# 4paradigm/OpenEmbedding

Hardware: NVIDIA H100
Metric: samples/sec (whole job, device-timed, max over ranks) deepfm Criteo dim 64 (higher is better)
Workload: dtype bf16

## Files before the change

openembedding_b200/csrc/cuda/gemm_wgmma.cu:

```cuda
#include <cuda.h>
#include <cuda_bf16.h>
#include <cuda_runtime.h>
#include "pdl.cuh"
#include <stdint.h>
#include <stdio.h>
#include <stdlib.h>
#include <string.h>

#include <string>
#include <vector>
#include <algorithm>

namespace {

constexpr int BM = 128, BK = 64;
constexpr int A_BYTES = BM * BK * 2;
template <int BN> constexpr int stages_for() { return BN == 64 ? 4 : 3; }
constexpr int NUM_CONSUMER_WARPS = 8;
constexpr int PRODUCER_WARP = NUM_CONSUMER_WARPS;
constexpr int NUM_THREADS = 32 * (NUM_CONSUMER_WARPS + 1);

enum EpiMode : int { EPI_FWD = 0, EPI_DX = 1, EPI_DW = 2, EPI_DX_FM = 3 };

struct GemmEpi {
    int mode, relu, ones_col, fm_cols;
    int M, N, D, mn_major;
    void* out; long long ldo;
    __nv_bfloat16* outT; long long ldoT;
    const __nv_bfloat16* mask; long long ldmask;
    const float* dlogit; const float* S; const float* emb; long long ldemb;
    int swap, mc;
    unsigned long long* dbg;
};

__device__ __forceinline__ uint32_t smem_u32(const void* p) { return (uint32_t)__cvta_generic_to_shared(p); }

__device__ __forceinline__ void mbar_init(uint64_t* b, uint32_t n) {
    asm volatile("mbarrier.init.shared::cta.b64 [%0], %1;" ::"r"(smem_u32(b)), "r"(n) : "memory");
}
__device__ __forceinline__ void mbar_expect_tx(uint64_t* b, uint32_t bytes) {
    asm volatile("mbarrier.arrive.expect_tx.shared::cta.b64 _, [%0], %1;" ::"r"(smem_u32(b)), "r"(bytes) : "memory");
}
__device__ __forceinline__ void mbar_arrive(uint64_t* b) {
    asm volatile("mbarrier.arrive.shared::cta.b64 _, [%0];" ::"r"(smem_u32(b)) : "memory");
}
__device__ __forceinline__ void mbar_arrive_cluster(uint64_t* b, uint32_t cta) {
    asm volatile("{\n\t.reg .b32 ra;\n\tmapa.shared::cluster.u32 ra, %0, %1;\n\t"
                 "mbarrier.arrive.release.cluster.shared::cluster.b64 _, [ra];\n\t}"
                 ::"r"(smem_u32(b)), "r"(cta) : "memory");
}
__device__ __forceinline__ bool mbar_try(uint64_t* b, uint32_t parity) {
    uint32_t ok;
    asm volatile("{\n\t.reg .pred p;\n\tmbarrier.try_wait.parity.shared::cta.b64 p, [%1], %2;\n\tselp.u32 %0, 1, 0, p;\n\t}"
                 : "=r"(ok) : "r"(smem_u32(b)), "r"(parity) : "memory");
    return ok != 0;
}
__device__ unsigned int g_pipeline_timeouts;
__device__ __forceinline__ bool mbar_wait(uint64_t* b, uint32_t parity) {
    for (uint32_t it = 0; it < (1u << 24); ++it)
        if (mbar_try(b, parity)) return true;
    atomicAdd(&g_pipeline_timeouts, 1u);
    return false;
}
__device__ __forceinline__ void tma_load_2d(void* smem_dst, const CUtensorMap* map, uint64_t* bar, int c0, int c1) {
    asm volatile("cp.async.bulk.tensor.2d.shared::cluster.global.mbarrier::complete_tx::bytes [%0], [%1, {%3, %4}], [%2];"
                 ::"r"(smem_u32(smem_dst)), "l"(map), "r"(smem_u32(bar)), "r"(c0), "r"(c1) : "memory");
}
__device__ __forceinline__ void tma_load_2d_mc(void* smem_dst, const CUtensorMap* map, uint64_t* bar, int c0, int c1, uint16_t mask) {
    asm volatile("cp.async.bulk.tensor.2d.shared::cluster.global.mbarrier::complete_tx::bytes.multicast::cluster [%0], [%1, {%4, %5}], [%2], %3;"
                 ::"r"(smem_u32(smem_dst)), "l"(map), "r"(smem_u32(bar)), "h"(mask), "r"(c0), "r"(c1) : "memory");
}
__device__ __forceinline__ void cluster_sync_all() {
    asm volatile("barrier.cluster.arrive.release.aligned;" ::: "memory");
    asm volatile("barrier.cluster.wait.acquire.aligned;" ::: "memory");
}
__device__ __forceinline__ void named_bar_sync(int id, int threads) {
    asm volatile("bar.sync %0, %1;" ::"r"(id), "r"(threads) : "memory");
}

__device__ __forceinline__ uint64_t gmma_desc(uint32_t smem_addr, uint32_t lbo_bytes) {
    uint64_t d = 0;
    d |= (uint64_t)((smem_addr & 0x3FFFFu) >> 4);
    d |= (uint64_t)((lbo_bytes >> 4) & 0x3FFFu) << 16;
    d |= (uint64_t)(1024 >> 4) << 32;
    d |= (uint64_t)1 << 62;
    return d;
}
__device__ __forceinline__ void wgmma_fence() { asm volatile("wgmma.fence.sync.aligned;" ::: "memory"); }
__device__ __forceinline__ void wgmma_commit() { asm volatile("wgmma.commit_group.sync.aligned;" ::: "memory"); }
template <int N>
__device__ __forceinline__ void wgmma_wait() { asm volatile("wgmma.wait_group.sync.aligned %0;" ::"n"(N) : "memory"); }
template <int R>
__device__ __forceinline__ void acc_fence(float (&d)[R]) {
#pragma unroll
    for (int i = 0; i < R; ++i) asm volatile("" : "+f"(d[i])::"memory");
}

template <int TRANS>
__device__ __forceinline__ void wgmma_n64(float (&d)[32], uint64_t da, uint64_t db, uint32_t scale_d) {
    asm volatile("{\n\t.reg .pred p;\n\tsetp.ne.b32 p, %34, 0;\n\t"
                 "wgmma.mma_async.sync.aligned.m64n64k16.f32.bf16.bf16 {"
                 "%0, %1, %2, %3, %4, %5, %6, %7, %8, %9, %10, %11, %12, %13, %14, %15, "
                 "%16, %17, %18, %19, %20, %21, %22, %23, %24, %25, %26, %27, %28, %29, %30, %31"
                 "}, %32, %33, p, 1, 1, %35, %35;\n\t}"
                 : "+f"(d[0]), "+f"(d[1]), "+f"(d[2]), "+f"(d[3]), "+f"(d[4]), "+f"(d[5]), "+f"(d[6]), "+f"(d[7]),
                   "+f"(d[8]), "+f"(d[9]), "+f"(d[10]), "+f"(d[11]), "+f"(d[12]), "+f"(d[13]), "+f"(d[14]), "+f"(d[15]),
                   "+f"(d[16]), "+f"(d[17]), "+f"(d[18]), "+f"(d[19]), "+f"(d[20]), "+f"(d[21]), "+f"(d[22]), "+f"(d[23]),
                   "+f"(d[24]), "+f"(d[25]), "+f"(d[26]), "+f"(d[27]), "+f"(d[28]), "+f"(d[29]), "+f"(d[30]), "+f"(d[31])
                 : "l"(da), "l"(db), "r"(scale_d), "n"(TRANS));
}
template <int TRANS>
__device__ __forceinline__ void wgmma_n128(float (&d)[64], uint64_t da, uint64_t db, uint32_t scale_d) {
    asm volatile("{\n\t.reg .pred p;\n\tsetp.ne.b32 p, %66, 0;\n\t"
                 "wgmma.mma_async.sync.aligned.m64n128k16.f32.bf16.bf16 {"
                 "%0, %1, %2, %3, %4, %5, %6, %7, %8, %9, %10, %11, %12, %13, %14, %15, "
                 "%16, %17, %18, %19, %20, %21, %22, %23, %24, %25, %26, %27, %28, %29, %30, %31, "
                 "%32, %33, %34, %35, %36, %37, %38, %39, %40, %41, %42, %43, %44, %45, %46, %47, "
                 "%48, %49, %50, %51, %52, %53, %54, %55, %56, %57, %58, %59, %60, %61, %62, %63"
                 "}, %64, %65, p, 1, 1, %67, %67;\n\t}"
                 : "+f"(d[0]), "+f"(d[1]), "+f"(d[2]), "+f"(d[3]), "+f"(d[4]), "+f"(d[5]), "+f"(d[6]), "+f"(d[7]),
                   "+f"(d[8]), "+f"(d[9]), "+f"(d[10]), "+f"(d[11]), "+f"(d[12]), "+f"(d[13]), "+f"(d[14]), "+f"(d[15]),
                   "+f"(d[16]), "+f"(d[17]), "+f"(d[18]), "+f"(d[19]), "+f"(d[20]), "+f"(d[21]), "+f"(d[22]), "+f"(d[23]),
                   "+f"(d[24]), "+f"(d[25]), "+f"(d[26]), "+f"(d[27]), "+f"(d[28]), "+f"(d[29]), "+f"(d[30]), "+f"(d[31]),
                   "+f"(d[32]), "+f"(d[33]), "+f"(d[34]), "+f"(d[35]), "+f"(d[36]), "+f"(d[37]), "+f"(d[38]), "+f"(d[39]),
                   "+f"(d[40]), "+f"(d[41]), "+f"(d[42]), "+f"(d[43]), "+f"(d[44]), "+f"(d[45]), "+f"(d[46]), "+f"(d[47]),
                   "+f"(d[48]), "+f"(d[49]), "+f"(d[50]), "+f"(d[51]), "+f"(d[52]), "+f"(d[53]), "+f"(d[54]), "+f"(d[55]),
                   "+f"(d[56]), "+f"(d[57]), "+f"(d[58]), "+f"(d[59]), "+f"(d[60]), "+f"(d[61]), "+f"(d[62]), "+f"(d[63])
                 : "l"(da), "l"(db), "r"(scale_d), "n"(TRANS));
}
template <int BN, int TRANS>
__device__ __forceinline__ void wgmma_stage(float (&acc)[BN / 2], uint32_t a0, uint32_t b0, int g, bool first) {
#pragma unroll
    for (int k = 0; k < BK / 16; ++k) {
        const uint64_t da = TRANS ? gmma_desc(a0 + g * 8192 + k * 2048, 8192) : gmma_desc(a0 + g * 8192 + k * 32, 16);
        const uint64_t db = TRANS ? gmma_desc(b0 + k * 2048, 8192) : gmma_desc(b0 + k * 32, 16);
        const uint32_t sd = (first && k == 0) ? 0u : 1u;
        if constexpr (BN == 64) wgmma_n64<TRANS>(acc, da, db, sd);
        else wgmma_n128<TRANS>(acc, da, db, sd);
    }
}

template <int BN>
__device__ __forceinline__ void mma_tile(float (&acc)[BN / 2], const uint8_t* sA, const uint8_t* sB, uint64_t* full,
                                         uint64_t* empty, int stages, uint32_t kiter, int nkb, bool mn_major, int g,
                                         int C) {
    constexpr int B_BYTES = BN * BK * 2;
    const int lane = threadIdx.x & 31;
#pragma unroll
    for (int j = 0; j < BN / 2; ++j) acc[j] = 0.f;
    auto release = [&](uint32_t it) {
        const int s = it % stages;
        if (C > 1) { if (lane < C) mbar_arrive_cluster(&empty[s], (uint32_t)lane); }
        else if (lane == 0) mbar_arrive(&empty[s]);
    };
    for (int i = 0; i < nkb; ++i) {
        const uint32_t it = kiter + i;
        const int s = it % stages;
        mbar_wait(&full[s], (it / stages) & 1u);
        const uint32_t a0 = smem_u32(sA + s * A_BYTES), b0 = smem_u32(sB + s * B_BYTES);
        wgmma_fence();
        if (mn_major) wgmma_stage<BN, 1>(acc, a0, b0, g, i == 0);
        else wgmma_stage<BN, 0>(acc, a0, b0, g, i == 0);
        wgmma_commit();
        if (i > 0) {
            wgmma_wait<1>();
            acc_fence(acc);
            release(it - 1);
        }
    }
    wgmma_wait<0>();
    acc_fence(acc);
    if (nkb > 0) release(kiter + nkb - 1);
}

template <int BN>
__device__ __forceinline__ void epilogue_tile(const GemmEpi& E, float (&acc)[BN / 2], int m_blk, int n_blk, int g,
                                              uint8_t* stage, int qstride, const CUtensorMap* tO, const CUtensorMap* tT) {
    const int mode = E.mode, relu = E.relu, ones_col = E.ones_col, fm_cols = E.fm_cols, N = E.N, D = E.D;
    const bool has_t = E.outT != nullptr;
    const int t = threadIdx.x & 127, w = t >> 5, l = t & 31;
    const bool f32out = (mode == EPI_DW || mode == EPI_DX_FM);
    const int q = 2 * g + (w >> 1);
    uint8_t* wstage = stage + q * qstride;
    uint8_t* tstage = wstage + BN * 128;
    constexpr int LOOK = BN == 64 ? 4 : 1;
#pragma unroll
    for (int i = 0; i < 2; ++i) {
        const int qrow = (w & 1) * 16 + (l >> 2) + 8 * i;
        const int row = m_blk * BM + q * 32 + qrow;
        const bool rv = row < E.M;
        const bool fm_row = mode == EPI_DX_FM && rv && n_blk * BN < fm_cols;
        const float dl = fm_row ? __ldg(E.dlogit + row) : 0.f;
        const __nv_bfloat16* mrow = E.mask + (size_t)row * E.ldmask;
        const float* erow = E.emb + (size_t)row * E.ldemb;
        const float* sb = E.S + (size_t)row * D;
#pragma unroll
        for (int j0 = 0; j0 < BN / 8; j0 += LOOK) {
            float4 v[LOOK];
#pragma unroll
            for (int jj = 0; jj < LOOK; ++jj) {
                const int n = n_blk * BN + 8 * (j0 + jj) + 2 * (l & 3);
                v[jj] = make_float4(0.f, 0.f, 0.f, 0.f);
                if (mode == EPI_DX) {
                    if (rv && n < N) {
                        const float2 mk = __bfloat1622float2(__ldg(reinterpret_cast<const __nv_bfloat162*>(mrow + n)));
                        v[jj].x = mk.x; v[jj].y = mk.y;
                    }
                } else if (fm_row && n < fm_cols) {
                    const float2 e2 = __ldg(reinterpret_cast<const float2*>(erow + n));
                    v[jj] = make_float4(e2.x, e2.y, __ldg(sb + n % D), __ldg(sb + (n + 1) % D));
                }
            }
#pragma unroll
            for (int jj = 0; jj < LOOK; ++jj) {
                const int j = j0 + jj;
                const int c = 8 * j + 2 * (l & 3);
                const int n = n_blk * BN + c;
                float x[2] = {acc[4 * j + 2 * i], acc[4 * j + 2 * i + 1]};
                if (mode == EPI_FWD) {
#pragma unroll
                    for (int u = 0; u < 2; ++u) {
                        if (relu) x[u] = fmaxf(x[u], 0.f);
                        if (n + u == ones_col) x[u] = 1.f;
                        if (n + u >= N) x[u] = 0.f;
                    }
                } else if (mode == EPI_DX) {
                    const float mv[2] = {v[jj].x, v[jj].y};
#pragma unroll
                    for (int u = 0; u < 2; ++u)
                        if (!rv || !(mv[u] > 0.f) || n + u == ones_col || n + u >= N) x[u] = 0.f;
                } else if (fm_row && n < fm_cols) {
                    x[0] += dl * (v[jj].z - v[jj].x);
                    x[1] += dl * (v[jj].w - v[jj].y);
                }
                if (f32out) {
                    const int cc = c & 31;
                    *reinterpret_cast<float2*>(wstage + (c >> 5) * 4096 + qrow * 128 + ((((cc >> 2) ^ (qrow & 7))) << 4) + (cc & 3) * 4) =
                        make_float2(x[0], x[1]);
                } else {
                    const int cc = c & 63;
                    *reinterpret_cast<__nv_bfloat162*>(wstage + (c >> 6) * 4096 + qrow * 128 + ((((cc >> 3) ^ (qrow & 7))) << 4) + (cc & 7) * 2) =
                        __floats2bfloat162_rn(x[0], x[1]);
                    if (has_t) {
                        *reinterpret_cast<__nv_bfloat16*>(tstage + c * 64 + qrow * 2) = __float2bfloat16_rn(x[0]);
                        *reinterpret_cast<__nv_bfloat16*>(tstage + (c + 1) * 64 + qrow * 2) = __float2bfloat16_rn(x[1]);
                    }
                }
            }
        }
    }
    asm volatile("fence.proxy.async.shared::cta;" ::: "memory");
    named_bar_sync(2 + g, 128);
    if (t == 0) {
        if (E.fm_cols != -7) {
#pragma unroll 1
            for (int qq = 2 * g; qq < 2 * g + 2; ++qq) {
                const int row0 = m_blk * BM + qq * 32;
                uint8_t* ws = stage + qq * qstride;
                if (f32out) {
#pragma unroll 1
                    for (int h = 0; h < BN / 32; ++h) {
                        const int n0 = n_blk * BN + 32 * h;
                        if (E.mode == EPI_DW)
                            asm volatile("cp.reduce.async.bulk.tensor.2d.global.shared::cta.add.tile.bulk_group [%0, {%2, %3}], [%1];"
                                         ::"l"(tO), "r"(smem_u32(ws + h * 4096)), "r"(n0), "r"(row0) : "memory");
                        else
                            asm volatile("cp.async.bulk.tensor.2d.global.shared::cta.bulk_group [%0, {%2, %3}], [%1];"
                                         ::"l"(tO), "r"(smem_u32(ws + h * 4096)), "r"(n0), "r"(row0) : "memory");
                    }
                } else {
#pragma unroll 1
                    for (int h = 0; h < BN / 64; ++h)
                        asm volatile("cp.async.bulk.tensor.2d.global.shared::cta.bulk_group [%0, {%2, %3}], [%1];"
                                     ::"l"(tO), "r"(smem_u32(ws + h * 4096)), "r"(n_blk * BN + 64 * h), "r"(row0) : "memory");
                    if (E.outT)
                        asm volatile("cp.async.bulk.tensor.2d.global.shared::cta.bulk_group [%0, {%2, %3}], [%1];"
                                     ::"l"(tT), "r"(smem_u32(ws + BN * 128)), "r"(row0), "r"(n_blk * BN) : "memory");
                }
            }
        }
        asm volatile("cp.async.bulk.commit_group;" ::: "memory");
    }
}

template <int BN>
__global__ void __launch_bounds__(NUM_THREADS, 2)
exb_gemm_wgmma_kernel(const __grid_constant__ CUtensorMap tmA, const __grid_constant__ CUtensorMap tmB,
                      const __grid_constant__ CUtensorMap tmO, const __grid_constant__ CUtensorMap tmT,
                      GemmEpi E, int num_k_blocks, int k_blocks_per_split) {
    static_assert(BN == 64 || BN == 128, "tile width");
    constexpr int STAGES = stages_for<BN>();
    constexpr int B_BYTES = BN * BK * 2;
    constexpr int QSTAGE = BN * 128 + BN * 64;
    static_assert(4 * QSTAGE <= STAGES * (A_BYTES + B_BYTES), "epilogue staging aliases the stage memory");
    extern __shared__ __align__(1024) uint8_t smem_raw[];
    uint8_t* smem = smem_raw + ((1024u - (smem_u32(smem_raw) & 1023u)) & 1023u);
    uint8_t* sA = smem;
    uint8_t* sB = smem + STAGES * A_BYTES;
    uint64_t* full = reinterpret_cast<uint64_t*>(sB + STAGES * B_BYTES);
    uint64_t* empty = full + STAGES;

    exb::pdl_trigger();
    const int warp = threadIdx.x >> 5, lane = threadIdx.x & 31;
    const int m_blk = E.swap ? blockIdx.y : blockIdx.x, n_blk = E.swap ? blockIdx.x : blockIdx.y;
    const bool dbg = E.dbg != nullptr && blockIdx.x == 0 && blockIdx.y == 0 && blockIdx.z == 0;
#define GSTAMP(i) do { if (dbg) { unsigned long long _t; asm volatile("mov.u64 %0, %%globaltimer;" : "=l"(_t)); E.dbg[i] = _t; } } while (0)
    if (threadIdx.x == 0) GSTAMP(0);
    const int kb0 = blockIdx.z * k_blocks_per_split;
    const int kb1 = min(num_k_blocks, kb0 + k_blocks_per_split);
    const int nkb = kb1 - kb0;
    const int C = E.mc > 1 ? E.mc : 1;
    uint32_t crank = 0;
    if (C > 1) asm volatile("mov.u32 %0, %%cluster_ctarank;" : "=r"(crank));
    const uint16_t cmask = (uint16_t)((1u << C) - 1u);

    if (threadIdx.x == 0) {
        for (int i = 0; i < STAGES; ++i) { mbar_init(&full[i], 1); mbar_init(&empty[i], (uint32_t)(NUM_CONSUMER_WARPS * C)); }
        asm volatile("fence.mbarrier_init.release.cluster;" ::: "memory");
        asm volatile("prefetch.tensormap [%0];" ::"l"(&tmA) : "memory");
        asm volatile("prefetch.tensormap [%0];" ::"l"(&tmB) : "memory");
    }
    __syncthreads();
    if (C > 1) cluster_sync_all();
    exb::pdl_wait();
    if (threadIdx.x == 0) GSTAMP(1);

    if (warp == PRODUCER_WARP) {
        if (lane == 0) {
            for (int i = 0; i < nkb; ++i) {
                const int s = i % STAGES;
                const uint32_t ph = (uint32_t)(i / STAGES) & 1u;
                mbar_wait(&empty[s], ph ^ 1u);
                mbar_expect_tx(&full[s], A_BYTES + B_BYTES);
                if (E.mn_major) {
                    if (C > 1) {
                        if (crank == 0) {
                            tma_load_2d_mc(sA + s * A_BYTES, &tmA, &full[s], m_blk * BM, (kb0 + i) * BK, cmask);
                            tma_load_2d_mc(sA + s * A_BYTES + A_BYTES / 2, &tmA, &full[s], m_blk * BM + 64, (kb0 + i) * BK, cmask);
                        }
                    } else {
                        tma_load_2d(sA + s * A_BYTES, &tmA, &full[s], m_blk * BM, (kb0 + i) * BK);
                        tma_load_2d(sA + s * A_BYTES + A_BYTES / 2, &tmA, &full[s], m_blk * BM + 64, (kb0 + i) * BK);
                    }
#pragma unroll
                    for (int h = 0; h < BN / 64; ++h)
                        tma_load_2d(sB + s * B_BYTES + h * 8192, &tmB, &full[s], n_blk * BN + 64 * h, (kb0 + i) * BK);
                    continue;
                }
                if (C > 1) {
                    if (crank == 0) tma_load_2d_mc(sA + s * A_BYTES, &tmA, &full[s], (kb0 + i) * BK, m_blk * BM, cmask);
                } else {
                    tma_load_2d(sA + s * A_BYTES, &tmA, &full[s], (kb0 + i) * BK, m_blk * BM);
                }
                tma_load_2d(sB + s * B_BYTES, &tmB, &full[s], (kb0 + i) * BK, n_blk * BN);
            }
        }
    } else {
        const int g = warp >> 2;
        float acc[BN / 2];
        if (dbg && threadIdx.x == 0 && nkb > 0) { mbar_wait(&full[0], 0); GSTAMP(2); }
        mma_tile<BN>(acc, sA, sB, full, empty, STAGES, 0u, nkb, E.mn_major != 0, g, C);
        if (threadIdx.x == 0) GSTAMP(3);
        named_bar_sync(1, 32 * NUM_CONSUMER_WARPS);
        epilogue_tile<BN>(E, acc, m_blk, n_blk, g, smem, QSTAGE, &tmO, &tmT);
        if ((threadIdx.x & 127) == 0) asm volatile("cp.async.bulk.wait_group.read 0;" ::: "memory");
        if (threadIdx.x == 0) GSTAMP(4);
    }
    __syncthreads();
    if (threadIdx.x == 0) GSTAMP(5);
    if (C > 1) cluster_sync_all();
}

constexpr int CH_STAGES = 3;
constexpr int CH_BN = 64;
constexpr int CH_B_BYTES = CH_BN * BK * 2;
constexpr int CH_MAX_PROB = 8;
constexpr int CH_MAX_MB = 64;

struct ChainMaps { CUtensorMap tmA, tmB, tmO; };
struct ChainMapsAll { ChainMaps m[CH_MAX_PROB]; };
struct ChainMeta {
    GemmEpi E;
    int m_tiles, n_tiles, splits, nkb, per;
    int item0, items;
    int dep, dep_kind, dep_need;
    int signal;
};

__device__ __forceinline__ void ch_decode(const ChainMeta* M, int nprob, int item, int& p, int& m, int& n, int& z) {
    p = 0;
#pragma unroll 1
    for (int i = 1; i < nprob; ++i)
        if (item >= M[i].item0) p = i;
    const int local = item - M[p].item0;
    const int mn = M[p].m_tiles * M[p].n_tiles;
    z = local / mn;
    const int r = local - z * mn;
    m = r / M[p].n_tiles;
    n = r - m * M[p].n_tiles;
}
__device__ __forceinline__ unsigned ch_ld_acquire(const unsigned* p) {
    unsigned v;
    asm volatile("ld.acquire.gpu.global.u32 %0, [%1];" : "=r"(v) : "l"(p) : "memory");
    return v;
}

__global__ void __launch_bounds__(NUM_THREADS, 2)
exb_gemm_chain_kernel(const __grid_constant__ ChainMapsAll MAPS, const ChainMeta* __restrict__ metas, int nprob, int total_items,
                      unsigned* __restrict__ ready, int* __restrict__ err) {
    const ChainMaps* maps = MAPS.m;
    extern __shared__ __align__(1024) uint8_t smem_raw[];
    uint8_t* smem = smem_raw + ((1024u - (smem_u32(smem_raw) & 1023u)) & 1023u);
    uint8_t* sA = smem;
    uint8_t* sB = smem + CH_STAGES * A_BYTES;
    uint8_t* sStage = sB + CH_STAGES * CH_B_BYTES;
    uint64_t* full = reinterpret_cast<uint64_t*>(sStage + 4 * 8192);
    uint64_t* empty = full + CH_STAGES;
    ChainMeta* M = reinterpret_cast<ChainMeta*>(empty + CH_STAGES);

    exb::pdl_trigger();
    const int warp = threadIdx.x >> 5, lane = threadIdx.x & 31;
    for (int i = threadIdx.x; i < nprob * (int)(sizeof(ChainMeta) / 4); i += blockDim.x)
        reinterpret_cast<uint32_t*>(M)[i] = reinterpret_cast<const uint32_t*>(metas)[i];
    if (threadIdx.x == 0) {
        for (int i = 0; i < CH_STAGES; ++i) { mbar_init(&full[i], 1); mbar_init(&empty[i], NUM_CONSUMER_WARPS); }
        asm volatile("fence.mbarrier_init.release.cluster;" ::: "memory");
    }
    __syncthreads();
    exb::pdl_wait();

    if (warp == PRODUCER_WARP) {
        if (lane == 0) {
            uint32_t kiter = 0;
            for (int item = blockIdx.x; item < total_items; item += gridDim.x) {
                int p, m_blk, n_blk, z;
                ch_decode(M, nprob, item, p, m_blk, n_blk, z);
                const ChainMeta& Q = M[p];
                const int kb0 = z * Q.per, kb1 = min(Q.nkb, kb0 + Q.per);
                if (Q.dep_kind) {
                    int mb0 = m_blk, mb1 = m_blk + 1;
                    if (Q.dep_kind == 2) { mb0 = (kb0 * BK) / BM; mb1 = (kb1 * BK + BM - 1) / BM; }
                    const unsigned* cnt = ready + Q.dep * CH_MAX_MB;
                    for (int mb = mb0; mb < mb1; ++mb) {
                        uint32_t it = 0;
                        while (ch_ld_acquire(cnt + mb) < (unsigned)Q.dep_need) {
                            __nanosleep(64);
                            if (++it > (1u << 22)) { atomicCAS(err, 0, 100 + p); break; }
                        }
                    }
                    asm volatile("fence.proxy.async;" ::: "memory");
                }
                const CUtensorMap* tA = &maps[p].tmA;
                const CUtensorMap* tB = &maps[p].tmB;
                for (int kb = kb0; kb < kb1; ++kb, ++kiter) {
                    const int s = kiter % CH_STAGES;
                    const uint32_t ph = (kiter / CH_STAGES) & 1u;
                    mbar_wait(&empty[s], ph ^ 1u);
                    mbar_expect_tx(&full[s], A_BYTES + CH_B_BYTES);
                    if (Q.E.mn_major) {
                        tma_load_2d(sA + s * A_BYTES, tA, &full[s], m_blk * BM, kb * BK);
                        tma_load_2d(sA + s * A_BYTES + A_BYTES / 2, tA, &full[s], m_blk * BM + 64, kb * BK);
                        tma_load_2d(sB + s * CH_B_BYTES, tB, &full[s], n_blk * CH_BN, kb * BK);
                    } else {
                        tma_load_2d(sA + s * A_BYTES, tA, &full[s], kb * BK, m_blk * BM);
                        tma_load_2d(sB + s * CH_B_BYTES, tB, &full[s], kb * BK, n_blk * CH_BN);
                    }
                }
            }
        }
    } else {
        const int g = warp >> 2;
        uint32_t kiter = 0;
        float acc[CH_BN / 2];
        for (int item = blockIdx.x; item < total_items; item += gridDim.x) {
            int p, m_blk, n_blk, z;
            ch_decode(M, nprob, item, p, m_blk, n_blk, z);
            const ChainMeta& Q = M[p];
            const int kb0 = z * Q.per, kb1 = min(Q.nkb, kb0 + Q.per);
            const int nk = __shfl_sync(0xffffffffu, kb1 - kb0, 0);
            const int mn = __shfl_sync(0xffffffffu, Q.E.mn_major, 0);
            mma_tile<CH_BN>(acc, sA, sB, full, empty, CH_STAGES, kiter, nk, mn != 0, g, 1);
            kiter += nk;
            epilogue_tile<CH_BN>(Q.E, acc, m_blk, n_blk, g, sStage, 8192, &maps[p].tmO, &maps[p].tmO);
            if ((threadIdx.x & 127) == 0) {
                if (Q.signal) {
                    asm volatile("cp.async.bulk.wait_group 0;" ::: "memory");
                    asm volatile("fence.proxy.async;" ::: "memory");
                    __threadfence();
                    atomicAdd(&ready[p * CH_MAX_MB + m_blk], 1u);
                } else {
                    asm volatile("cp.async.bulk.wait_group.read 0;" ::: "memory");
                }
            }
            named_bar_sync(2 + g, 128);
        }
    }
    __syncthreads();
    if (warp == 0) {
        unsigned last = 0;
        if (lane == 0) {
            __threadfence();
            last = (atomicAdd(&ready[CH_MAX_PROB * CH_MAX_MB], 1u) == gridDim.x - 1) ? 1u : 0u;
        }
        last = __shfl_sync(0xffffffffu, last, 0);
        if (last) {
            for (int i = lane; i < CH_MAX_PROB * CH_MAX_MB; i += 32) ready[i] = 0u;
            __syncwarp();
            if (lane == 0) { __threadfence(); ready[CH_MAX_PROB * CH_MAX_MB] = 0u; }
        }
    }
}

typedef CUresult (*EncodeTiledFn)(CUtensorMap*, CUtensorMapDataType, cuuint32_t, void*, const cuuint64_t*,
                                  const cuuint64_t*, const cuuint32_t*, const cuuint32_t*, CUtensorMapInterleave,
                                  CUtensorMapSwizzle, CUtensorMapL2promotion, CUtensorMapFloatOOBfill);
EncodeTiledFn g_encode = nullptr;
thread_local std::string g_gemm_err;

bool make_map_ex(CUtensorMap* map, CUtensorMapDataType dt, int esize, const void* ptr, long long rows, long long cols,
                 long long ld, int box_cols, int box_rows, CUtensorMapSwizzle sw);

bool make_map(CUtensorMap* map, const void* ptr, long long rows, long long cols, long long ld, int box_rows) {
    return make_map_ex(map, CU_TENSOR_MAP_DATA_TYPE_BFLOAT16, 2, ptr, rows, cols, ld, BK, box_rows, CU_TENSOR_MAP_SWIZZLE_128B);
}

bool make_map_ex(CUtensorMap* map, CUtensorMapDataType dt, int esize, const void* ptr, long long rows, long long cols,
                 long long ld, int box_cols, int box_rows, CUtensorMapSwizzle sw) {
    if (!g_encode) {
        void* fn = nullptr;
        cudaDriverEntryPointQueryResult qres;
        if (cudaGetDriverEntryPoint("cuTensorMapEncodeTiled", &fn, cudaEnableDefault, &qres) != cudaSuccess || !fn) {
            g_gemm_err = "cuTensorMapEncodeTiled entry point not found";
            return false;
        }
        g_encode = (EncodeTiledFn)fn;
    }
    cuuint64_t dims[2] = {(cuuint64_t)cols, (cuuint64_t)rows};
    cuuint64_t strides[1] = {(cuuint64_t)ld * esize};
    cuuint32_t box[2] = {(cuuint32_t)box_cols, (cuuint32_t)box_rows};
    cuuint32_t estr[2] = {1, 1};
    CUresult r = g_encode(map, dt, 2, const_cast<void*>(ptr), dims, strides, box, estr,
                          CU_TENSOR_MAP_INTERLEAVE_NONE, sw, CU_TENSOR_MAP_L2_PROMOTION_L2_128B,
                          CU_TENSOR_MAP_FLOAT_OOB_FILL_NONE);
    if (r != CUDA_SUCCESS) {
        g_gemm_err = "cuTensorMapEncodeTiled failed: " + std::to_string((int)r);
        return false;
    }
    return true;
}

template <int BN>
constexpr size_t gemm_smem() { return stages_for<BN>() * (A_BYTES + BN * BK * 2) + (2 * stages_for<BN>() + 1) * 8 + 16 + 1024; }

int pick_swap() {
    static int v = -1;
    if (v < 0) { const char* e = getenv("EXB_GEMM_SWAP"); v = e ? atoi(e) : 0; }
    return v;
}
int pick_bn(int M, int N, int K) {
    static int forced = -1;
    if (forced < 0) { const char* e = getenv("EXB_GEMM_BN"); forced = e ? atoi(e) : 0; }
    if (forced == 64 || forced == 128) return forced;
    if (K <= 128 && N >= 512 && M >= 8192) return 128;
    return 64;
}

template <int BN>
cudaError_t launch_gemm(dim3 grid, cudaStream_t stream, const CUtensorMap& tmA, const CUtensorMap& tmB, const CUtensorMap& tmO,
                        const CUtensorMap& tmT, const GemmEpi& E, int nkb, int per) {
    static bool attr_set = false;
    if (!attr_set) {
        cudaFuncSetAttribute(exb_gemm_wgmma_kernel<BN>, cudaFuncAttributeMaxDynamicSharedMemorySize, (int)gemm_smem<BN>());
        attr_set = true;
    }
    if (E.mc > 1) {
        cudaLaunchConfig_t cfg = {};
        cfg.gridDim = grid; cfg.blockDim = dim3(NUM_THREADS); cfg.dynamicSmemBytes = gemm_smem<BN>(); cfg.stream = stream;
        cudaLaunchAttribute attr[2];
        attr[0].id = cudaLaunchAttributeClusterDimension;
        attr[0].val.clusterDim.x = 1; attr[0].val.clusterDim.y = (unsigned)E.mc; attr[0].val.clusterDim.z = 1;
        attr[1].id = cudaLaunchAttributeProgrammaticStreamSerialization;
        attr[1].val.programmaticStreamSerializationAllowed = 1;
        cfg.attrs = attr; cfg.numAttrs = exb::pdl_enabled() ? 2 : 1;
        return cudaLaunchKernelEx(&cfg, exb_gemm_wgmma_kernel<BN>, tmA, tmB, tmO, tmT, E, nkb, per);
    }
    return exb::launch_pdl(exb_gemm_wgmma_kernel<BN>, grid, dim3(NUM_THREADS), gemm_smem<BN>(), stream, tmA, tmB, tmO, tmT,
                           E, nkb, per);
}

int pick_mc(int n_tiles) {
    static int lim = -1;
    if (lim < 0) { const char* e = getenv("EXB_GEMM_MC"); lim = e ? atoi(e) : 0; }
    if (lim <= 1 || pick_swap()) return 1;
    int best = 1;
    for (int c = 2; c <= 8 && c <= lim; ++c)
        if (n_tiles % c == 0) best = c;
    return best;
}

}

extern "C" {

const char* exb_gemm_last_error() { return g_gemm_err.c_str(); }

int exb_gemm_timeouts() {
    unsigned v = 0, z = 0;
    if (cudaDeviceSynchronize() != cudaSuccess || cudaMemcpyFromSymbol(&v, g_pipeline_timeouts, sizeof(v)) != cudaSuccess ||
        cudaMemcpyToSymbol(g_pipeline_timeouts, &z, sizeof(z)) != cudaSuccess) return -1;
    return (int)v;
}

int exb_gemm_bf16_nt(uint64_t A, long long lda, uint64_t B, long long ldb, int M, int N, int K, int mode, int relu,
                     int ones_col, uint64_t out, long long ldo, uint64_t outT, long long ldoT, uint64_t mask,
                     long long ldmask, uint64_t dlogit, uint64_t S, uint64_t emb, long long ldemb, int fm_cols, int D,
                     int splits, uint64_t stream, uint64_t dbg) {
    if (K % BK != 0 || lda % 8 != 0 || ldb % 8 != 0) { g_gemm_err = "gemm: K %% 64 / ld %% 8 violated"; return -1; }
    CUtensorMap tmA, tmB;
    if (!make_map(&tmA, (const void*)A, M, K, lda, BM)) return -1;
    const int BN = pick_bn(M, N, K);
    if (!make_map(&tmB, (const void*)B, N, K, ldb, BN)) return -1;
    CUtensorMap tmO, tmT;
    const bool f32out = (mode == EPI_DW || mode == EPI_DX_FM);
    if (f32out) {
        if (!make_map_ex(&tmO, CU_TENSOR_MAP_DATA_TYPE_FLOAT32, 4, (const void*)out, M, N, ldo, 32, 32, CU_TENSOR_MAP_SWIZZLE_128B)) return -1;
    } else {
        if (!make_map_ex(&tmO, CU_TENSOR_MAP_DATA_TYPE_BFLOAT16, 2, (const void*)out, M, (N + 63) / 64 * 64, ldo, 64, 32, CU_TENSOR_MAP_SWIZZLE_128B)) return -1;
    }
    tmT = tmO;
    if (outT && !make_map_ex(&tmT, CU_TENSOR_MAP_DATA_TYPE_BFLOAT16, 2, (const void*)outT, (N + 63) / 64 * 64, M, ldoT, 32, BN, CU_TENSOR_MAP_SWIZZLE_NONE)) return -1;
    GemmEpi E;
    E.mode = mode; E.relu = relu; E.ones_col = ones_col; E.fm_cols = fm_cols; E.M = M; E.N = N; E.D = D > 0 ? D : 1; E.mn_major = 0;
    E.out = (void*)out; E.ldo = ldo; E.outT = (__nv_bfloat16*)outT; E.ldoT = ldoT;
    E.mask = (const __nv_bfloat16*)mask; E.ldmask = ldmask;
    E.dlogit = (const float*)dlogit; E.S = (const float*)S; E.emb = (const float*)emb; E.ldemb = ldemb;
    E.dbg = (unsigned long long*)dbg;
    const int nkb = K / BK;
    if (splits < 1) splits = 1;
    if (splits > nkb) splits = nkb;
    const int per = (nkb + splits - 1) / splits;
    splits = (nkb + per - 1) / per;
    dim3 grid((M + BM - 1) / BM, (N + BN - 1) / BN, splits);
    E.swap = pick_swap(); E.mc = pick_mc((int)grid.y);
    if (E.swap) grid = dim3(grid.y, grid.x, grid.z);
    cudaError_t err = BN == 128 ? launch_gemm<128>(grid, (cudaStream_t)stream, tmA, tmB, tmO, tmT, E, nkb, per)
                                : launch_gemm<64>(grid, (cudaStream_t)stream, tmA, tmB, tmO, tmT, E, nkb, per);
    if (err == cudaSuccess) err = cudaGetLastError();
    if (err != cudaSuccess) { g_gemm_err = std::string("gemm launch: ") + cudaGetErrorString(err); return -1; }
    return 0;
}

int exb_gemm_bf16_tn(uint64_t A, long long lda, uint64_t B, long long ldb, int M, int N, int K, uint64_t out,
                     long long ldo, int splits, uint64_t stream) {
    if (K % BK != 0 || lda % 8 != 0 || ldb % 8 != 0) { g_gemm_err = "gemm_tn: K %% 64 / ld %% 8 violated"; return -1; }
    CUtensorMap tmA, tmB, tmO, tmT;
    if (!make_map_ex(&tmA, CU_TENSOR_MAP_DATA_TYPE_BFLOAT16, 2, (const void*)A, K, M, lda, 64, BK, CU_TENSOR_MAP_SWIZZLE_128B)) return -1;
    if (!make_map_ex(&tmB, CU_TENSOR_MAP_DATA_TYPE_BFLOAT16, 2, (const void*)B, K, N, ldb, 64, BK, CU_TENSOR_MAP_SWIZZLE_128B)) return -1;
    if (!make_map_ex(&tmO, CU_TENSOR_MAP_DATA_TYPE_FLOAT32, 4, (const void*)out, M, N, ldo, 32, 32, CU_TENSOR_MAP_SWIZZLE_128B)) return -1;
    tmT = tmO;
    GemmEpi E;
    memset(&E, 0, sizeof(E));
    E.mode = EPI_DW; E.ones_col = -1; E.M = M; E.N = N; E.D = 1; E.mn_major = 1;
    E.out = (void*)out; E.ldo = ldo;
    const int BN = pick_bn(M, N, K);
    const int nkb = K / BK;
    if (splits < 1) splits = 1;
    if (splits > nkb) splits = nkb;
    const int per = (nkb + splits - 1) / splits;
    splits = (nkb + per - 1) / per;
    dim3 grid((M + BM - 1) / BM, (N + BN - 1) / BN, splits);
    E.swap = pick_swap(); E.mc = pick_mc((int)grid.y);
    if (E.swap) grid = dim3(grid.y, grid.x, grid.z);
    cudaError_t err = BN == 128 ? launch_gemm<128>(grid, (cudaStream_t)stream, tmA, tmB, tmO, tmT, E, nkb, per)
                                : launch_gemm<64>(grid, (cudaStream_t)stream, tmA, tmB, tmO, tmT, E, nkb, per);
    if (err == cudaSuccess) err = cudaGetLastError();
    if (err != cudaSuccess) { g_gemm_err = std::string("gemm_tn launch: ") + cudaGetErrorString(err); return -1; }
    return 0;
}

struct ChainDesc {
    int tn;
    int M, N, K;
    unsigned long long A, B, out;
    long long lda, ldb, ldo;
    int mode, relu, ones_col, fm_cols, D, splits;
    unsigned long long mask; long long ldmask;
    unsigned long long dlogit, S, emb; long long ldemb;
    int dep, dep_kind;
};
struct Chain {
    int nprob = 0, total = 0, grid = 0;
    ChainMapsAll maps;
    ChainMeta* d_meta = nullptr;
    unsigned* d_ready = nullptr;
    int* d_err = nullptr;
    size_t smem = 0;
};

int exb_chain_desc_size() { return (int)sizeof(ChainDesc); }

void* exb_chain_create(const void* descs, int n, int sms) {
    if (n < 1 || n > CH_MAX_PROB) { g_gemm_err = "chain: 1..8 GEMMs"; return nullptr; }
    const ChainDesc* D = reinterpret_cast<const ChainDesc*>(descs);
    std::vector<ChainMaps> maps(n);
    std::vector<ChainMeta> meta(n);
    int item0 = 0;
    for (int i = 0; i < n; ++i) {
        const ChainDesc& d = D[i];
        ChainMeta& Q = meta[i];
        memset(&Q, 0, sizeof(Q));
        if (d.K % BK != 0 || d.lda % 8 != 0 || d.ldb % 8 != 0) { g_gemm_err = "chain: K % 64 / ld % 8 violated"; return nullptr; }
        GemmEpi& E = Q.E;
        E.mode = d.tn ? EPI_DW : d.mode; E.relu = d.relu; E.ones_col = d.tn ? -1 : d.ones_col; E.fm_cols = d.fm_cols;
        E.M = d.M; E.N = d.N; E.D = d.D > 0 ? d.D : 1; E.mn_major = d.tn ? 1 : 0;
        E.out = (void*)d.out; E.ldo = d.ldo; E.outT = nullptr; E.ldoT = 0;
        E.mask = (const __nv_bfloat16*)d.mask; E.ldmask = d.ldmask;
        E.dlogit = (const float*)d.dlogit; E.S = (const float*)d.S; E.emb = (const float*)d.emb; E.ldemb = d.ldemb;
        E.swap = 0; E.mc = 1; E.dbg = nullptr;
        const bool f32out = (E.mode == EPI_DW || E.mode == EPI_DX_FM);
        bool ok;
        if (d.tn) {
            ok = make_map_ex(&maps[i].tmA, CU_TENSOR_MAP_DATA_TYPE_BFLOAT16, 2, (const void*)d.A, d.K, d.M, d.lda, 64, BK, CU_TENSOR_MAP_SWIZZLE_128B) &&
                 make_map_ex(&maps[i].tmB, CU_TENSOR_MAP_DATA_TYPE_BFLOAT16, 2, (const void*)d.B, d.K, d.N, d.ldb, 64, BK, CU_TENSOR_MAP_SWIZZLE_128B);
        } else {
            ok = make_map(&maps[i].tmA, (const void*)d.A, d.M, d.K, d.lda, BM) && make_map(&maps[i].tmB, (const void*)d.B, d.N, d.K, d.ldb, CH_BN);
        }
        if (ok) {
            if (f32out) ok = make_map_ex(&maps[i].tmO, CU_TENSOR_MAP_DATA_TYPE_FLOAT32, 4, (const void*)d.out, d.M, d.N, d.ldo, 32, 32, CU_TENSOR_MAP_SWIZZLE_128B);
            else ok = make_map_ex(&maps[i].tmO, CU_TENSOR_MAP_DATA_TYPE_BFLOAT16, 2, (const void*)d.out, d.M, (d.N + 63) / 64 * 64, d.ldo, 64, 32, CU_TENSOR_MAP_SWIZZLE_128B);
        }
        if (!ok) return nullptr;
        Q.nkb = d.K / BK;
        int splits = d.tn ? std::max(1, d.splits) : 1;
        if (splits > Q.nkb) splits = Q.nkb;
        Q.per = (Q.nkb + splits - 1) / splits;
        Q.splits = (Q.nkb + Q.per - 1) / Q.per;
        Q.m_tiles = (d.M + BM - 1) / BM; Q.n_tiles = (d.N + CH_BN - 1) / CH_BN;
        Q.item0 = item0; Q.items = Q.m_tiles * Q.n_tiles * Q.splits;
        item0 += Q.items;
        Q.dep = d.dep; Q.dep_kind = d.dep >= 0 ? d.dep_kind : 0; Q.dep_need = 0; Q.signal = 0;
        if (Q.dep_kind) {
            if (d.dep >= i) { g_gemm_err = "chain: a GEMM may only depend on an earlier one"; return nullptr; }
            meta[d.dep].signal = 1;
            Q.dep_need = (NUM_CONSUMER_WARPS / 4) * meta[d.dep].n_tiles;
            if (meta[d.dep].m_tiles > CH_MAX_MB) { g_gemm_err = "chain: too many row blocks"; return nullptr; }
        }
    }
    Chain* c = new Chain();
    c->nprob = n; c->total = item0;
    c->smem = CH_STAGES * (A_BYTES + CH_B_BYTES) + 4 * 8192 + 2 * CH_STAGES * 8 + CH_MAX_PROB * sizeof(ChainMeta) + 1024;
    cudaFuncSetAttribute(exb_gemm_chain_kernel, cudaFuncAttributeMaxDynamicSharedMemorySize, (int)c->smem);
    cudaFuncSetAttribute(exb_gemm_chain_kernel, cudaFuncAttributePreferredSharedMemoryCarveout, 100);
    int occ = (2 * (c->smem + 1024) <= 232448) ? 2 : 1;
    if (const char* ev = getenv("EXB_CHAIN_CTAS_PER_SM")) occ = std::max(1, std::min(2, atoi(ev)));
    c->grid = std::min(c->total, (sms > 0 ? sms : 132) * occ);
    memset(&c->maps, 0, sizeof(c->maps));
    for (int i = 0; i < n; ++i) c->maps.m[i] = maps[i];
    if (cudaMalloc(&c->d_meta, n * sizeof(ChainMeta)) != cudaSuccess ||
        cudaMalloc(&c->d_ready, (CH_MAX_PROB * CH_MAX_MB + 32) * 4) != cudaSuccess || cudaMalloc(&c->d_err, 4) != cudaSuccess) {
        g_gemm_err = "chain: cudaMalloc failed"; delete c; return nullptr;
    }
    cudaMemcpy(c->d_meta, meta.data(), n * sizeof(ChainMeta), cudaMemcpyHostToDevice);
    cudaMemset(c->d_ready, 0, (CH_MAX_PROB * CH_MAX_MB + 32) * 4);
    cudaMemset(c->d_err, 0, 4);
    return c;
}
void exb_chain_destroy(void* h) {
    Chain* c = (Chain*)h;
    cudaFree(c->d_meta); cudaFree(c->d_ready); cudaFree(c->d_err);
    delete c;
}
int exb_chain_launch(void* h, uint64_t stream) {
    Chain* c = (Chain*)h;
    cudaError_t err = exb::launch_pdl(exb_gemm_chain_kernel, dim3(c->grid), dim3(NUM_THREADS), c->smem, (cudaStream_t)stream,
                              c->maps, (const ChainMeta*)c->d_meta, c->nprob, c->total, c->d_ready, c->d_err);
    if (err == cudaSuccess) err = cudaGetLastError();
    if (err != cudaSuccess) { g_gemm_err = std::string("chain launch: ") + cudaGetErrorString(err); return -1; }
    return 0;
}
int exb_chain_status(void* h) {
    Chain* c = (Chain*)h;
    int v = 0;
    cudaDeviceSynchronize();
    cudaMemcpy(&v, c->d_err, 4, cudaMemcpyDeviceToHost);
    return v;
}
int exb_chain_info(void* h, int* out) { Chain* c = (Chain*)h; out[0] = c->total; out[1] = c->grid; out[2] = (int)c->smem; return 0; }

}
```

Before: 12.71 million.

## TMA-prefetch epilogue mask and embedding tiles into shared staging buffers

After: 13.10 million, median of 6. 1.03x the previous value.

```diff
diff --git a/openembedding_b200/csrc/cuda/gemm_wgmma.cu b/openembedding_b200/csrc/cuda/gemm_wgmma.cu
--- a/openembedding_b200/csrc/cuda/gemm_wgmma.cu
+++ b/openembedding_b200/csrc/cuda/gemm_wgmma.cu
@@ -174,6 +174,26 @@
 }
 
 template <int BN>
+__device__ __forceinline__ int epi_src_boxes(int mode, int fm_cols, int N, int n_blk) {
+    const int n0 = n_blk * BN;
+    if (mode == EPI_DX) return min(BN / 64, (N - n0 + 63) / 64);
+    if (mode == EPI_DX_FM && fm_cols > n0) return min(BN / 32, (fm_cols - n0 + 31) / 32);
+    return 0;
+}
+template <int BN>
+__device__ __forceinline__ void load_epi_src(const CUtensorMap* tE, uint64_t* bar, uint8_t* stage, int qstride, int g,
+                                             int m_blk, int n_blk, int boxes, int M, bool f32) {
+    const int row0 = m_blk * BM + 2 * g * 32;
+    const int quarters = row0 >= M ? 0 : (row0 + 32 >= M ? 1 : 2);
+    mbar_expect_tx(bar, (uint32_t)(quarters * boxes * 4096));
+#pragma unroll 1
+    for (int qq = 0; qq < quarters; ++qq)
+#pragma unroll 1
+        for (int h = 0; h < boxes; ++h)
+            tma_load_2d(stage + (2 * g + qq) * qstride + h * 4096, tE, bar, n_blk * BN + (f32 ? 32 : 64) * h, row0 + 32 * qq);
+}
+
+template <int BN>
 __device__ __forceinline__ void epilogue_tile(const GemmEpi& E, float (&acc)[BN / 2], int m_blk, int n_blk, int g,
                                               uint8_t* stage, int qstride, const CUtensorMap* tO, const CUtensorMap* tT) {
     const int mode = E.mode, relu = E.relu, ones_col = E.ones_col, fm_cols = E.fm_cols, N = E.N, D = E.D;
@@ -183,7 +203,7 @@
     const int q = 2 * g + (w >> 1);
     uint8_t* wstage = stage + q * qstride;
     uint8_t* tstage = wstage + BN * 128;
-    constexpr int LOOK = BN == 64 ? 4 : 1;
+    constexpr int SG = BN == 64 ? BN / 8 : 2;
 #pragma unroll
     for (int i = 0; i < 2; ++i) {
         const int qrow = (w & 1) * 16 + (l >> 2) + 8 * i;
@@ -191,32 +211,26 @@
         const bool rv = row < E.M;
         const bool fm_row = mode == EPI_DX_FM && rv && n_blk * BN < fm_cols;
         const float dl = fm_row ? __ldg(E.dlogit + row) : 0.f;
-        const __nv_bfloat16* mrow = E.mask + (size_t)row * E.ldmask;
-        const float* erow = E.emb + (size_t)row * E.ldemb;
         const float* sb = E.S + (size_t)row * D;
 #pragma unroll
-        for (int j0 = 0; j0 < BN / 8; j0 += LOOK) {
-            float4 v[LOOK];
-#pragma unroll
-            for (int jj = 0; jj < LOOK; ++jj) {
+        for (int j0 = 0; j0 < BN / 8; j0 += SG) {
+            float2 s[SG];
+#pragma unroll
+            for (int jj = 0; jj < SG; ++jj) {
                 const int n = n_blk * BN + 8 * (j0 + jj) + 2 * (l & 3);
-                v[jj] = make_float4(0.f, 0.f, 0.f, 0.f);
-                if (mode == EPI_DX) {
-                    if (rv && n < N) {
-                        const float2 mk = __bfloat1622float2(__ldg(reinterpret_cast<const __nv_bfloat162*>(mrow + n)));
-                        v[jj].x = mk.x; v[jj].y = mk.y;
-                    }
-                } else if (fm_row && n < fm_cols) {
-                    const float2 e2 = __ldg(reinterpret_cast<const float2*>(erow + n));
-                    v[jj] = make_float4(e2.x, e2.y, __ldg(sb + n % D), __ldg(sb + (n + 1) % D));
-                }
+                s[jj] = make_float2(0.f, 0.f);
+                if (fm_row && n < fm_cols) s[jj] = make_float2(__ldg(sb + n % D), __ldg(sb + (n + 1) % D));
             }
 #pragma unroll
-            for (int jj = 0; jj < LOOK; ++jj) {
+            for (int jj = 0; jj < SG; ++jj) {
                 const int j = j0 + jj;
                 const int c = 8 * j + 2 * (l & 3);
                 const int n = n_blk * BN + c;
                 float x[2] = {acc[4 * j + 2 * i], acc[4 * j + 2 * i + 1]};
+                const int cc = f32out ? (c & 31) : (c & 63);
+                uint8_t* slot = f32out
+                    ? wstage + (c >> 5) * 4096 + qrow * 128 + ((((cc >> 2) ^ (qrow & 7))) << 4) + (cc & 3) * 4
+                    : wstage + (c >> 6) * 4096 + qrow * 128 + ((((cc >> 3) ^ (qrow & 7))) << 4) + (cc & 7) * 2;
                 if (mode == EPI_FWD) {
 #pragma unroll
                     for (int u = 0; u < 2; ++u) {
@@ -225,22 +239,21 @@
                         if (n + u >= N) x[u] = 0.f;
                     }
                 } else if (mode == EPI_DX) {
-                    const float mv[2] = {v[jj].x, v[jj].y};
+                    float2 mk = make_float2(0.f, 0.f);
+                    if (rv && n < N) mk = __bfloat1622float2(*reinterpret_cast<const __nv_bfloat162*>(slot));
+                    const float mv[2] = {mk.x, mk.y};
 #pragma unroll
                     for (int u = 0; u < 2; ++u)
                         if (!rv || !(mv[u] > 0.f) || n + u == ones_col || n + u >= N) x[u] = 0.f;
                 } else if (fm_row && n < fm_cols) {
-                    x[0] += dl * (v[jj].z - v[jj].x);
-                    x[1] += dl * (v[jj].w - v[jj].y);
+                    const float2 e = *reinterpret_cast<const float2*>(slot);
+                    x[0] += dl * (s[jj].x - e.x);
+                    x[1] += dl * (s[jj].y - e.y);
                 }
                 if (f32out) {
-                    const int cc = c & 31;
-                    *reinterpret_cast<float2*>(wstage + (c >> 5) * 4096 + qrow * 128 + ((((cc >> 2) ^ (qrow & 7))) << 4) + (cc & 3) * 4) =
-                        make_float2(x[0], x[1]);
+                    *reinterpret_cast<float2*>(slot) = make_float2(x[0], x[1]);
                 } else {
-                    const int cc = c & 63;
-                    *reinterpret_cast<__nv_bfloat162*>(wstage + (c >> 6) * 4096 + qrow * 128 + ((((cc >> 3) ^ (qrow & 7))) << 4) + (cc & 7) * 2) =
-                        __floats2bfloat162_rn(x[0], x[1]);
+                    *reinterpret_cast<__nv_bfloat162*>(slot) = __floats2bfloat162_rn(x[0], x[1]);
                     if (has_t) {
                         *reinterpret_cast<__nv_bfloat16*>(tstage + c * 64 + qrow * 2) = __float2bfloat16_rn(x[0]);
                         *reinterpret_cast<__nv_bfloat16*>(tstage + (c + 1) * 64 + qrow * 2) = __float2bfloat16_rn(x[1]);
@@ -287,7 +300,7 @@
 __global__ void __launch_bounds__(NUM_THREADS, 2)
 exb_gemm_wgmma_kernel(const __grid_constant__ CUtensorMap tmA, const __grid_constant__ CUtensorMap tmB,
                       const __grid_constant__ CUtensorMap tmO, const __grid_constant__ CUtensorMap tmT,
-                      GemmEpi E, int num_k_blocks, int k_blocks_per_split) {
+                      const __grid_constant__ CUtensorMap tmE, GemmEpi E, int num_k_blocks, int k_blocks_per_split) {
     static_assert(BN == 64 || BN == 128, "tile width");
     constexpr int STAGES = stages_for<BN>();
     constexpr int B_BYTES = BN * BK * 2;
@@ -299,6 +312,7 @@
     uint8_t* sB = smem + STAGES * A_BYTES;
     uint64_t* full = reinterpret_cast<uint64_t*>(sB + STAGES * B_BYTES);
     uint64_t* empty = full + STAGES;
+    uint64_t* srcfull = empty + STAGES;
 
     exb::pdl_trigger();
     const int warp = threadIdx.x >> 5, lane = threadIdx.x & 31;
@@ -316,6 +330,7 @@
 
     if (threadIdx.x == 0) {
         for (int i = 0; i < STAGES; ++i) { mbar_init(&full[i], 1); mbar_init(&empty[i], (uint32_t)(NUM_CONSUMER_WARPS * C)); }
+        mbar_init(&srcfull[0], 1); mbar_init(&srcfull[1], 1);
         asm volatile("fence.mbarrier_init.release.cluster;" ::: "memory");
         asm volatile("prefetch.tensormap [%0];" ::"l"(&tmA) : "memory");
         asm volatile("prefetch.tensormap [%0];" ::"l"(&tmB) : "memory");
@@ -362,6 +377,12 @@
         mma_tile<BN>(acc, sA, sB, full, empty, STAGES, 0u, nkb, E.mn_major != 0, g, C);
         if (threadIdx.x == 0) GSTAMP(3);
         named_bar_sync(1, 32 * NUM_CONSUMER_WARPS);
+        const int boxes = epi_src_boxes<BN>(E.mode, E.fm_cols, E.N, n_blk);
+        if (boxes) {
+            if ((threadIdx.x & 127) == 0)
+                load_epi_src<BN>(&tmE, &srcfull[g], smem, QSTAGE, g, m_blk, n_blk, boxes, E.M, E.mode == EPI_DX_FM);
+            mbar_wait(&srcfull[g], 0);
+        }
         epilogue_tile<BN>(E, acc, m_blk, n_blk, g, smem, QSTAGE, &tmO, &tmT);
         if ((threadIdx.x & 127) == 0) asm volatile("cp.async.bulk.wait_group.read 0;" ::: "memory");
         if (threadIdx.x == 0) GSTAMP(4);
@@ -377,7 +398,7 @@
 constexpr int CH_MAX_PROB = 8;
 constexpr int CH_MAX_MB = 64;
 
-struct ChainMaps { CUtensorMap tmA, tmB, tmO; };
+struct ChainMaps { CUtensorMap tmA, tmB, tmO, tmE; };
 struct ChainMapsAll { ChainMaps m[CH_MAX_PROB]; };
 struct ChainMeta {
     GemmEpi E;
@@ -416,7 +437,9 @@
     uint8_t* sStage = sB + CH_STAGES * CH_B_BYTES;
     uint64_t* full = reinterpret_cast<uint64_t*>(sStage + 4 * 8192);
     uint64_t* empty = full + CH_STAGES;
-    ChainMeta* M = reinterpret_cast<ChainMeta*>(empty + CH_STAGES);
+    uint64_t* sfree = empty + CH_STAGES;
+    uint64_t* srcfull = sfree + 2;
+    ChainMeta* M = reinterpret_cast<ChainMeta*>(srcfull + 2);
 
     exb::pdl_trigger();
     const int warp = threadIdx.x >> 5, lane = threadIdx.x & 31;
@@ -424,6 +447,7 @@
         reinterpret_cast<uint32_t*>(M)[i] = reinterpret_cast<const uint32_t*>(metas)[i];
     if (threadIdx.x == 0) {
         for (int i = 0; i < CH_STAGES; ++i) { mbar_init(&full[i], 1); mbar_init(&empty[i], NUM_CONSUMER_WARPS); }
+        for (int i = 0; i < 2; ++i) { mbar_init(&sfree[i], 1); mbar_init(&srcfull[i], 1); }
         asm volatile("fence.mbarrier_init.release.cluster;" ::: "memory");
     }
     __syncthreads();
@@ -431,8 +455,8 @@
 
     if (warp == PRODUCER_WARP) {
         if (lane == 0) {
-            uint32_t kiter = 0;
-            for (int item = blockIdx.x; item < total_items; item += gridDim.x) {
+            uint32_t kiter = 0, tile = 0;
+            for (int item = blockIdx.x; item < total_items; item += gridDim.x, ++tile) {
                 int p, m_blk, n_blk, z;
                 ch_decode(M, nprob, item, p, m_blk, n_blk, z);
                 const ChainMeta& Q = M[p];
@@ -452,7 +476,16 @@
                 }
                 const CUtensorMap* tA = &maps[p].tmA;
                 const CUtensorMap* tB = &maps[p].tmB;
+                const int boxes = epi_src_boxes<CH_BN>(Q.E.mode, Q.E.fm_cols, Q.E.N, n_blk);
+                const int handoff = kb0 + min(CH_STAGES, kb1 - kb0 - 1);
                 for (int kb = kb0; kb < kb1; ++kb, ++kiter) {
+                    if (kb == handoff) {
+                        if (tile > 0) { mbar_wait(&sfree[0], (tile - 1) & 1u); mbar_wait(&sfree[1], (tile - 1) & 1u); }
+                        if (boxes)
+                            for (int g = 0; g < 2; ++g)
+                                load_epi_src<CH_BN>(&maps[p].tmE, &srcfull[g], sStage, 8192, g, m_blk, n_blk, boxes, Q.E.M,
+                                                    Q.E.mode == EPI_DX_FM);
+                    }
                     const int s = kiter % CH_STAGES;
                     const uint32_t ph = (kiter / CH_STAGES) & 1u;
                     mbar_wait(&empty[s], ph ^ 1u);
@@ -470,7 +503,7 @@
         }
     } else {
         const int g = warp >> 2;
-        uint32_t kiter = 0;
+        uint32_t kiter = 0, nsrc = 0;
         float acc[CH_BN / 2];
         for (int item = blockIdx.x; item < total_items; item += gridDim.x) {
             int p, m_blk, n_blk, z;
@@ -481,6 +514,7 @@
             const int mn = __shfl_sync(0xffffffffu, Q.E.mn_major, 0);
             mma_tile<CH_BN>(acc, sA, sB, full, empty, CH_STAGES, kiter, nk, mn != 0, g, 1);
             kiter += nk;
+            if (epi_src_boxes<CH_BN>(Q.E.mode, Q.E.fm_cols, Q.E.N, n_blk)) mbar_wait(&srcfull[g], (nsrc++) & 1u);
             epilogue_tile<CH_BN>(Q.E, acc, m_blk, n_blk, g, sStage, 8192, &maps[p].tmO, &maps[p].tmO);
             if ((threadIdx.x & 127) == 0) {
                 if (Q.signal) {
@@ -491,6 +525,7 @@
                 } else {
                     asm volatile("cp.async.bulk.wait_group.read 0;" ::: "memory");
                 }
+                mbar_arrive(&sfree[g]);
             }
             named_bar_sync(2 + g, 128);
         }
@@ -550,7 +585,24 @@
 }
 
 template <int BN>
-constexpr size_t gemm_smem() { return stages_for<BN>() * (A_BYTES + BN * BK * 2) + (2 * stages_for<BN>() + 1) * 8 + 16 + 1024; }
+constexpr size_t gemm_smem() { return stages_for<BN>() * (A_BYTES + BN * BK * 2) + (2 * stages_for<BN>() + 2) * 8 + 16 + 1024; }
+
+bool make_epi_src_map(CUtensorMap* map, int mode, int fm_cols, int M, int N, const void* mask, long long ldmask,
+                      const void* emb, long long ldemb) {
+    const bool dx = mode == EPI_DX, fm = mode == EPI_DX_FM && fm_cols > 0;
+    if (!dx && !fm) return true;
+    const void* p = dx ? mask : emb;
+    const long long ld = dx ? ldmask : ldemb;
+    const int esize = dx ? 2 : 4;
+    if (!p) { g_gemm_err = dx ? "gemm: EPI_DX needs the relu mask" : "gemm: fm_cols > 0 needs the embedding rows"; return false; }
+    if (((uintptr_t)p & 15) != 0 || (ld * esize) % 16 != 0) {
+        g_gemm_err = dx ? "gemm: relu mask base / row stride not 16-byte aligned"
+                        : "gemm: embedding rows base / row stride not 16-byte aligned";
+        return false;
+    }
+    if (dx) return make_map_ex(map, CU_TENSOR_MAP_DATA_TYPE_BFLOAT16, 2, p, M, N, ld, 64, 32, CU_TENSOR_MAP_SWIZZLE_128B);
+    return make_map_ex(map, CU_TENSOR_MAP_DATA_TYPE_FLOAT32, 4, p, M, fm_cols, ld, 32, 32, CU_TENSOR_MAP_SWIZZLE_128B);
+}
 
 int pick_swap() {
     static int v = -1;
@@ -567,7 +619,7 @@
 
 template <int BN>
 cudaError_t launch_gemm(dim3 grid, cudaStream_t stream, const CUtensorMap& tmA, const CUtensorMap& tmB, const CUtensorMap& tmO,
-                        const CUtensorMap& tmT, const GemmEpi& E, int nkb, int per) {
+                        const CUtensorMap& tmT, const CUtensorMap& tmE, const GemmEpi& E, int nkb, int per) {
     static bool attr_set = false;
     if (!attr_set) {
         cudaFuncSetAttribute(exb_gemm_wgmma_kernel<BN>, cudaFuncAttributeMaxDynamicSharedMemorySize, (int)gemm_smem<BN>());
@@ -582,10 +634,10 @@
         attr[1].id = cudaLaunchAttributeProgrammaticStreamSerialization;
         attr[1].val.programmaticStreamSerializationAllowed = 1;
         cfg.attrs = attr; cfg.numAttrs = exb::pdl_enabled() ? 2 : 1;
-        return cudaLaunchKernelEx(&cfg, exb_gemm_wgmma_kernel<BN>, tmA, tmB, tmO, tmT, E, nkb, per);
+        return cudaLaunchKernelEx(&cfg, exb_gemm_wgmma_kernel<BN>, tmA, tmB, tmO, tmT, tmE, E, nkb, per);
     }
     return exb::launch_pdl(exb_gemm_wgmma_kernel<BN>, grid, dim3(NUM_THREADS), gemm_smem<BN>(), stream, tmA, tmB, tmO, tmT,
-                           E, nkb, per);
+                           tmE, E, nkb, per);
 }
 
 int pick_mc(int n_tiles) {
@@ -628,6 +680,8 @@
         if (!make_map_ex(&tmO, CU_TENSOR_MAP_DATA_TYPE_BFLOAT16, 2, (const void*)out, M, (N + 63) / 64 * 64, ldo, 64, 32, CU_TENSOR_MAP_SWIZZLE_128B)) return -1;
     }
     tmT = tmO;
+    CUtensorMap tmE = tmO;
+    if (!make_epi_src_map(&tmE, mode, fm_cols, M, N, (const void*)mask, ldmask, (const void*)emb, ldemb)) return -1;
     if (outT && !make_map_ex(&tmT, CU_TENSOR_MAP_DATA_TYPE_BFLOAT16, 2, (const void*)outT, (N + 63) / 64 * 64, M, ldoT, 32, BN, CU_TENSOR_MAP_SWIZZLE_NONE)) return -1;
     GemmEpi E;
     E.mode = mode; E.relu = relu; E.ones_col = ones_col; E.fm_cols = fm_cols; E.M = M; E.N = N; E.D = D > 0 ? D : 1; E.mn_major = 0;
@@ -643,8 +697,8 @@
     dim3 grid((M + BM - 1) / BM, (N + BN - 1) / BN, splits);
     E.swap = pick_swap(); E.mc = pick_mc((int)grid.y);
     if (E.swap) grid = dim3(grid.y, grid.x, grid.z);
-    cudaError_t err = BN == 128 ? launch_gemm<128>(grid, (cudaStream_t)stream, tmA, tmB, tmO, tmT, E, nkb, per)
-                                : launch_gemm<64>(grid, (cudaStream_t)stream, tmA, tmB, tmO, tmT, E, nkb, per);
+    cudaError_t err = BN == 128 ? launch_gemm<128>(grid, (cudaStream_t)stream, tmA, tmB, tmO, tmT, tmE, E, nkb, per)
+                                : launch_gemm<64>(grid, (cudaStream_t)stream, tmA, tmB, tmO, tmT, tmE, E, nkb, per);
     if (err == cudaSuccess) err = cudaGetLastError();
     if (err != cudaSuccess) { g_gemm_err = std::string("gemm launch: ") + cudaGetErrorString(err); return -1; }
     return 0;
@@ -653,11 +707,11 @@
 int exb_gemm_bf16_tn(uint64_t A, long long lda, uint64_t B, long long ldb, int M, int N, int K, uint64_t out,
                      long long ldo, int splits, uint64_t stream) {
     if (K % BK != 0 || lda % 8 != 0 || ldb % 8 != 0) { g_gemm_err = "gemm_tn: K %% 64 / ld %% 8 violated"; return -1; }
-    CUtensorMap tmA, tmB, tmO, tmT;
+    CUtensorMap tmA, tmB, tmO, tmT, tmE;
     if (!make_map_ex(&tmA, CU_TENSOR_MAP_DATA_TYPE_BFLOAT16, 2, (const void*)A, K, M, lda, 64, BK, CU_TENSOR_MAP_SWIZZLE_128B)) return -1;
     if (!make_map_ex(&tmB, CU_TENSOR_MAP_DATA_TYPE_BFLOAT16, 2, (const void*)B, K, N, ldb, 64, BK, CU_TENSOR_MAP_SWIZZLE_128B)) return -1;
     if (!make_map_ex(&tmO, CU_TENSOR_MAP_DATA_TYPE_FLOAT32, 4, (const void*)out, M, N, ldo, 32, 32, CU_TENSOR_MAP_SWIZZLE_128B)) return -1;
-    tmT = tmO;
+    tmT = tmE = tmO;
     GemmEpi E;
     memset(&E, 0, sizeof(E));
     E.mode = EPI_DW; E.ones_col = -1; E.M = M; E.N = N; E.D = 1; E.mn_major = 1;
@@ -671,8 +725,8 @@
     dim3 grid((M + BM - 1) / BM, (N + BN - 1) / BN, splits);
     E.swap = pick_swap(); E.mc = pick_mc((int)grid.y);
     if (E.swap) grid = dim3(grid.y, grid.x, grid.z);
-    cudaError_t err = BN == 128 ? launch_gemm<128>(grid, (cudaStream_t)stream, tmA, tmB, tmO, tmT, E, nkb, per)
-                                : launch_gemm<64>(grid, (cudaStream_t)stream, tmA, tmB, tmO, tmT, E, nkb, per);
+    cudaError_t err = BN == 128 ? launch_gemm<128>(grid, (cudaStream_t)stream, tmA, tmB, tmO, tmT, tmE, E, nkb, per)
+                                : launch_gemm<64>(grid, (cudaStream_t)stream, tmA, tmB, tmO, tmT, tmE, E, nkb, per);
     if (err == cudaSuccess) err = cudaGetLastError();
     if (err != cudaSuccess) { g_gemm_err = std::string("gemm_tn launch: ") + cudaGetErrorString(err); return -1; }
     return 0;
@@ -729,6 +783,8 @@
             if (f32out) ok = make_map_ex(&maps[i].tmO, CU_TENSOR_MAP_DATA_TYPE_FLOAT32, 4, (const void*)d.out, d.M, d.N, d.ldo, 32, 32, CU_TENSOR_MAP_SWIZZLE_128B);
             else ok = make_map_ex(&maps[i].tmO, CU_TENSOR_MAP_DATA_TYPE_BFLOAT16, 2, (const void*)d.out, d.M, (d.N + 63) / 64 * 64, d.ldo, 64, 32, CU_TENSOR_MAP_SWIZZLE_128B);
         }
+        if (ok && !d.tn)
+            ok = make_epi_src_map(&maps[i].tmE, E.mode, d.fm_cols, d.M, d.N, (const void*)d.mask, d.ldmask, (const void*)d.emb, d.ldemb);
         if (!ok) return nullptr;
         Q.nkb = d.K / BK;
         int splits = d.tn ? std::max(1, d.splits) : 1;
@@ -748,7 +804,7 @@
     }
     Chain* c = new Chain();
     c->nprob = n; c->total = item0;
-    c->smem = CH_STAGES * (A_BYTES + CH_B_BYTES) + 4 * 8192 + 2 * CH_STAGES * 8 + CH_MAX_PROB * sizeof(ChainMeta) + 1024;
+    c->smem = CH_STAGES * (A_BYTES + CH_B_BYTES) + 4 * 8192 + (2 * CH_STAGES + 4) * 8 + CH_MAX_PROB * sizeof(ChainMeta) + 1024;
     cudaFuncSetAttribute(exb_gemm_chain_kernel, cudaFuncAttributeMaxDynamicSharedMemorySize, (int)c->smem);
     cudaFuncSetAttribute(exb_gemm_chain_kernel, cudaFuncAttributePreferredSharedMemoryCarveout, 100);
     int occ = (2 * (c->smem + 1024) <= 232448) ? 2 : 1;
```
